# JessicaLeu-code/MotionPlanning_5D_m

Hardware: AMD Instinct MI355X
Metric: CFS iterations/sec, 5-DoF 30-wp 8-obs batch-1024; l_inf wp err vs quadprog (higher is better)
Workload: dtype f64

## Files before the change

### motionplanning_5d_m_amd/csrc/cfs_fused.hip

```cpp
#include "cfs_geom_dev.h"
#include <algorithm>
#include <atomic>
#include <type_traits>

namespace {

#define STAMP_IF(k) if (P.stamps) { const unsigned long long t_ = clock64(); if (tid == 0) s_acc[k] += t_ - t0_; t0_ = t_; }
#define STAMP(k) do { STAMP_IF(k) } while (0)

constexpr int CERT_AT = 6;
#ifndef CFS_WG_PER_CU
#define CFS_WG_PER_CU 1
#endif
constexpr double REF_A = 1e-4;
constexpr double REF_B = 1e-9;
constexpr int MV_BATCH = 16;
#ifndef CFS_TU
#define CFS_TU 8
#endif
#ifndef CFS_PR
#define CFS_PR 64
#endif
static_assert(CFS_PR % 8 == 0 && CFS_PR >= 8, "register-resident P columns come in chunks of 8");
constexpr int FT = 256;
// ... 209 lines not shown
}

template <int PR, int QB>
struct PRow {
    static constexpr int TU = CFS_TU;
    double v[PR];
    __device__ __forceinline__ void zero(double *ptail, int a, int q)
    {
#pragma unroll
        for (int b = 0; b < PR; ++b) v[b] = 0.0;
        for (int b = PR; b < q; ++b) ptail[(b - PR) * QB + a] = 0.0;
    }
    __device__ __forceinline__ double dot(const double *vec, const double *ptail, int a, int q) const
    {
        double s = 0.0;
#pragma unroll
        for (int b0 = 0; b0 < PR; b0 += 8)
            if (b0 < q) {
#pragma unroll
                for (int jj = 0; jj < 8; ++jj) s += v[b0 + jj] * vec[b0 + jj];
                __builtin_amdgcn_sched_barrier(0);
            }
        int b = PR;
        for (; b + TU <= q; b += TU) {
            double t[TU];
#pragma unroll
            for (int jj = 0; jj < TU; ++jj) t[jj] = ptail[(b + jj - PR) * QB + a];
#pragma unroll
            for (int jj = 0; jj < TU; ++jj) s += t[jj] * vec[b + jj];
        }
        for (; b < q; ++b) s += ptail[(b - PR) * QB + a] * vec[b];
        return s;
    }
    __device__ __forceinline__ void axpy(double alpha, const double *vec, double *ptail, int a, int q)
    {
#pragma unroll
        for (int b0 = 0; b0 < PR; b0 += 8)
            if (b0 < q) {
#pragma unroll
                for (int jj = 0; jj < 8; ++jj) v[b0 + jj] += alpha * vec[b0 + jj];
                __builtin_amdgcn_sched_barrier(0);
            }
        int b = PR;
        for (; b + TU <= q; b += TU) {
            double t[TU];
#pragma unroll
            for (int jj = 0; jj < TU; ++jj) t[jj] = ptail[(b + jj - PR) * QB + a];
#pragma unroll
            for (int jj = 0; jj < TU; ++jj) ptail[(b + jj - PR) * QB + a] = t[jj] + alpha * vec[b + jj];
        }
        for (; b < q; ++b) ptail[(b - PR) * QB + a] += alpha * vec[b];
    }
    __device__ __forceinline__ void axpy_mask(double alpha, const double *vec, const double *mask, double *ptail, int a, int q)
    {
#pragma unroll
        for (int b0 = 0; b0 < PR; b0 += 8)
            if (b0 < q) {
#pragma unroll
                for (int jj = 0; jj < 8; ++jj) v[b0 + jj] = (v[b0 + jj] + alpha * vec[b0 + jj]) * mask[b0 + jj];
                __builtin_amdgcn_sched_barrier(0);
            }
        int b = PR;
        for (; b + TU <= q; b += TU) {
            double t[TU];
#pragma unroll
            for (int jj = 0; jj < TU; ++jj) t[jj] = ptail[(b + jj - PR) * QB + a];
#pragma unroll
            for (int jj = 0; jj < TU; ++jj) ptail[(b + jj - PR) * QB + a] = (t[jj] + alpha * vec[b + jj]) * mask[b + jj];
        }
        for (; b < q; ++b) ptail[(b - PR) * QB + a] = (ptail[(b - PR) * QB + a] + alpha * vec[b]) * mask[b];
    }
    __device__ __forceinline__ void set_scaled(double alpha, const double *vec, double *ptail, int a, int q)
    {
#pragma unroll
        for (int b0 = 0; b0 < PR; b0 += 8)
            if (b0 < q) {
#pragma unroll
                for (int jj = 0; jj < 8; ++jj) v[b0 + jj] = alpha * vec[b0 + jj];
                __builtin_amdgcn_sched_barrier(0);
            }
        for (int b = PR; b < q; ++b) ptail[(b - PR) * QB + a] = alpha * vec[b];
    }
    __device__ __forceinline__ void store(double *dst, const double *ptail, int a, int q) const
    {
#pragma unroll
        for (int b0 = 0; b0 < PR; b0 += 8)
            if (b0 < q) {
#pragma unroll
                for (int jj = 0; jj < 8; ++jj) dst[b0 + jj] = v[b0 + jj];
                __builtin_amdgcn_sched_barrier(0);
            }
        int b = PR;
        for (; b + TU <= q; b += TU) {
            double t[TU];
#pragma unroll
            for (int jj = 0; jj < TU; ++jj) t[jj] = ptail[(b + jj - PR) * QB + a];
#pragma unroll
            for (int jj = 0; jj < TU; ++jj) dst[b + jj] = t[jj];
        }
        for (; b < q; ++b) dst[b] = ptail[(b - PR) * QB + a];
    }
};

struct FusedLayout {
    int rb, ob, x, u, qu, g, rhs, xs, up, wb, zb, d, r, rho, lam, prow, act, fre, prev, flag, slot, code, red, small, mx, racc, cost, ptail, lin, y, total_fixed;
};
__host__ __device__ inline FusedLayout fused_layout(int NJ, int H, int nobs, int QB, int PR)
{
    FusedLayout L;
    const int HN = H * NJ, NS = 2 * NJ;
    int o = 0;
    L.rb = o; o += (int)(sizeof(DevRobot) / 8);
    L.ob = o; o += nobs * 6;
    L.x = o; o += H * NS;
    L.u = o; o += HN;
    L.qu = o; o += HN;
    L.g = o; o += nobs * HN;
    L.rhs = o; o += nobs * H;
    L.xs = o; o += 3 * HN;
    L.up = o; o += HN;
    L.act = o; o += (QB + 1) / 2;
    L.fre = o; o += (QB + 1) / 2;
    L.prev = o; o += (QB + 1) / 2;
    L.flag = o; o += (nobs * H + 4 * HN + 7) / 8;
    L.code = o; o += (nobs * H + 4 * HN + 1) / 2;
    L.red = o; o += 64;
    L.small = o; o += 4 * NJ + nobs;
    L.mx = o; o += HN;
    L.racc = o; o += HN;
    L.cost = o; o += (int)(sizeof(DevCost) / 8);
    o = (o + 1) & ~1;
    L.lin = o;
    L.wb = o; o += 3 * HN;
    L.zb = o; o += 3 * HN;
    L.d = o; o += QB;
    L.r = o; o += QB;
    L.rho = o; o += QB;
    L.lam = o; o += QB;
    L.prow = o; o += QB;
    L.slot = o; o += (nobs * H + 4 * HN + 3) / 4;
    L.ptail = o;
    o = (o + 1) & ~1;
    L.y = o;
    L.total_fixed = o;
    return L;
}

template <int NJ, int QB, bool IDENT, bool JAC, class... Soft>
__global__ __launch_bounds__(FT, CFS_WG_PER_CU) void cfs_solve_fused_kernel(FusedParams P, Soft... soft_params)
{
    constexpr bool SOFT = sizeof...(Soft) > 0;
    static_assert(!SOFT || (sizeof...(Soft) == 1 && (std::is_same_v<Soft, SoftParams> && ...)), "Soft is empty or SoftParams");
    const SoftParams S{soft_params...};
    constexpr int NS = 2 * NJ, NVT = nvt(NJ), NE = 2 * NJ + 1;
    extern __shared__ __attribute__((aligned(16))) double lds[];
    const int b = P.order ? P.order[blockIdx.x] : (int)blockIdx.x, tid = threadIdx.x;
    const int H = P.H, nobs = P.nobs, HN = H * NJ, nn = HN, NX = H * NS;
    const double dt = P.dt;
    constexpr int PR = QB < CFS_PR ? QB : CFS_PR;
    const FusedLayout L = fused_layout(NJ, H, nobs, QB, PR);
    DevRobot *rb = reinterpret_cast<DevRobot *>(lds + L.rb);
    double *s_ob = lds + L.ob, *s_x = lds + L.x, *s_u = lds + L.u, *s_qu = lds + L.qu, *s_g = lds + L.g;
    double *s_rhs = lds + L.rhs, *xs = lds + L.xs, *s_up = lds + L.up, *wb = lds + L.wb, *zb = lds + L.zb;
    double *s_d = lds + L.d, *s_r = lds + L.r, *s_rho = lds + L.rho, *s_lam = lds + L.lam, *s_prow = lds + L.prow;
    int *s_act = reinterpret_cast<int *>(lds + L.act);
    int *s_free = reinterpret_cast<int *>(lds + L.fre);
    int *s_prev = reinterpret_cast<int *>(lds + L.prev);
    unsigned char *s_flag = reinterpret_cast<unsigned char *>(lds + L.flag);
    unsigned short *s_slot = reinterpret_cast<unsigned short *>(lds + L.slot);
    int *s_code = reinterpret_cast<int *>(lds + L.code);
    double *red_base = lds + L.red;
    int red_sel = 0;
#define red (red_base + 24 * (red_sel ^= 1))
    double *s_lim = lds + L.small, *s_v0 = s_lim + NJ, *s_th0 = s_v0 + NJ, *s_margin = s_th0 + 2 * NJ;
    double *s_mx = lds + L.mx;
    double *s_racc = lds + L.racc;
    int pool_slot;
    {
        int *pubp = reinterpret_cast<int *>(red_base + 63);
        if (tid == 0) {
            int sidx = (int)(((blockIdx.x * 0x9E3779B1u) >> 8) % (unsigned)P.pool_n);
            int probes = 0;
            while (atomicCAS(&P.pool_flag[sidx * 16], 0, 1) != 0) {
                sidx = sidx + 1 == P.pool_n ? 0 : sidx + 1;
                __builtin_amdgcn_s_sleep(2);
                if (++probes > (1 << 22)) { sidx = -1; break; }
            }
            pubp[0] = sidx;
        }
        __syncthreads();
        pool_slot = pubp[0];
        if (pool_slot < 0) {
            if (tid == 0 && P.piece == 0) { P.status[b] = CFS_NUMERIC; P.iter_O[b] = 1; P.total_iter[b] = 0; }
            return;
        }
    }
    double *const s_pt = P.Pt + (size_t)pool_slot * P.pt_stride;
    double *s_Y = lds + L.y;
    const int QY = P.qy;
    double *const Yg = P.Yg + (size_t)pool_slot * nn * nn;
    auto drop_pool = [&]() {
        __syncthreads();
        if (tid == 0) { __threadfence(); atomicExch(&P.pool_flag[pool_slot * 16], 0); }
    };
    const int ncon = nobs * H + (P.has_bounds ? 4 : 2) * HN;
    const int maxit = 8 * nn + 200;
    for (int e = tid; e < ncon; e += FT) {
        int code;
        if (e < nobs * H) { const int j = e / H; code = mk_code(CT_COL, e - j * H, j); }
        else {
            const int f2 = e - nobs * H, ty = f2 / HN, k = f2 - ty * HN, i = k / NJ;
            code = mk_code(1 + ty, i, k - i * NJ);
        }
        s_code[e] = code;
    }

    {
        const double *src = reinterpret_cast<const double *>(P.rb);
        for (int e = tid; e < (int)(sizeof(DevRobot) / 8); e += FT) lds[L.rb + e] = src[e];
        for (int e = tid; e < nobs * 6; e += FT) s_ob[e] = P.obs[(size_t)b * nobs * 6 + e];
        for (int e = tid; e < NX; e += FT) s_x[e] = P.x_init[(size_t)b * NX + e];
        for (int e = tid; e < HN; e += FT) { s_u[e] = 0.0; s_qu[e] = 0.0; s_mx[e] = P.has_bounds ? P.maxin[e] : 0.0; }
        if (tid < NJ) {
            s_lim[tid] = P.lim[tid];
            s_v0[tid] = P.xR1[(size_t)b * NS + NJ + tid];
            s_th0[tid] = P.xR1[(size_t)b * NS + tid];
        }
        if (tid < nobs) s_margin[tid] = P.margin[tid];
        if (P.cost) {
            const double *csrc = reinterpret_cast<const double *>(P.cost);
            for (int e = tid; e < (int)(sizeof(DevCost) / 8); e += FT) lds[L.cost + e] = csrc[e];
        }
    }
    __syncthreads();
    if (P.has_bounds)
        for (int e = tid; e < HN; e += FT) {
            const int i = e / NJ, c = e - i * NJ;
            double acc = 0.0;
            for (int k = 0; k <= i; ++k) acc += ((double)(i - k) + 0.5) * s_mx[k * NJ + c];
            s_racc[e] = (dt * dt) * acc;
        }
    unsigned long long *s_acc = reinterpret_cast<unsigned long long *>(red_base + 48);
    if (tid < 12) s_acc[tid] = 0ull;
    unsigned long long t0_ = P.stamps ? clock64() : 0ull;
    double cost_new = P.caug[b], cost_old = 100000.0;
    int iter_O = 1, total_iter = 0, noise_row = 0, status = CFS_OK_MAXITER;
    bool done = false;
    const double iw = S.inv_weight;
    int n_soft = 0;
    bool last_soft = false;
    const int nseg = nobs - P.nmesh;
    int launched = 0;
    if (P.resume) {
        for (int e = tid; e < NX; e += FT) s_x[e] = P.x_[(size_t)b * NX + e];
        for (int e = tid; e < HN; e += FT) { s_u[e] = P.u[(size_t)b * nn + e]; s_qu[e] = P.st_qu[(size_t)b * nn + e]; }
        cost_new = P.st_cost[2 * b]; cost_old = P.st_cost[2 * b + 1];
        iter_O = P.iter_O[b]; total_iter = P.total_iter[b]; status = P.status[b];
        noise_row = P.st_noise[b]; done = P.st_done[b] != 0;
        __syncthreads();
    } else if (P.piece == 0) {
        double d2 = 0.0;
        for (int e = tid; e < NX; e += FT) { const double v = s_x[e] - 1.0; d2 += v * v; }
        d2 = block_sum(d2, red, tid);
        if (sqrt(d2) < P.epsilon_O) { done = true; status = CFS_OK_CONVERGED; }
        else if (iter_O > P.max_o_iter) { done = true; status = CFS_OK_MAXITER; }
    } else if (P.piece == 2) {
        for (int e = tid; e < HN; e += FT) s_u[e] = P.u[(size_t)b * nn + e];
        __syncthreads();
    }

    PRow<PR, QB> Pr;
    int prev_q = 0;

    while (!done) {
        bool skip = false;
        if (P.piece == 0 && P.mode == CFS_MODE_PSGCFS) {
            skip = fabs(cost_new - cost_old) < 1e-4;
            if (!skip) cost_old = cost_new;
        } else if (P.piece == 0) cost_old = cost_new;
        const int noise_row_now = noise_row;
        if (P.piece == 0 && P.mode == CFS_MODE_PSGCFS && !skip) ++noise_row;
        auto prep = [&](int ph) {
            if (P.piece == 1) return;
            if (ph == 0) { for (int k = tid; k < HN; k += FT) xs[k] = s_u[k]; }
            else if (ph == 1) roll_lds<NJ>(xs, H, dt, tid);
            else if (ph == 2) {
                const bool psg = P.piece == 0 && P.mode == CFS_MODE_PSGCFS;
                const double sc = (double)iter_O * (double)iter_O + 1.0;
                const bool have = P.noise != nullptr && noise_row_now < P.noise_rows;
                for (int k = tid; k < HN; k += FT) {
                    s_up[k] = xs[2 * HN + k];
                    double v;
                    if (psg && skip) v = s_u[k];
                    else if (psg) {
                        const double nz = have ? P.noise[((size_t)b * P.noise_rows + noise_row_now) * nn + k] : 0.0;
                        v = s_u[k] - P.alpha * ((s_qu[k] + P.ff[(size_t)b * nn + k]) + 10.0 * nz / sc);
                    } else v = P.x0[(size_t)b * nn + k];
                    xs[k] = v;
                }
            } else roll_lds<NJ>(xs, H, dt, tid);
        };
        bool prepped = false;
        if constexpr (JAC) {
            if (nseg > 0) {
                const int W = P.lin_w;
                double *s_sc = lds + L.lin;
                double *s_en = s_sc + W * NJ * 6;
                double *s_tw = s_en + W * NJ * 6;
                double *s_bd = s_en + W * NVT * 6;
                for (int w0 = 0; w0 < H; w0 += W) {
                    const int Wc = min(W, H - w0);
                    if (w0 == 0) prep(0);
                    for (int e = tid; e < Wc * NJ; e += FT) {
                        const int m = e % NJ, wi = e / NJ;
                        double x = s_x[(w0 + wi) * NS + m];
                        x = x - rb->th_off[m];
                        double sn, cs;
                        sincos(x, &sn, &cs);
                        s_sc[e * 2] = sn;
                        s_sc[e * 2 + 1] = cs;
                    }
                    __syncthreads();
                    for (int wi = tid; wi < Wc; wi += FT) arm_chain(rb, NJ, s_sc + wi * NJ * 2, s_en + wi * NJ * 6, s_tw + wi * NJ * 6);
                    if (w0 == 0) prep(1);
                    __syncthreads();
                    STAMP(10);
                    for (int e = tid; e < NJ * Wc * nseg; e += FT) {
                        const int j = e % nseg, wi = (e / nseg) % Wc, k0 = e / (nseg * Wc);
                        s_bd[(wi * NJ + k0) * nseg + j] = seg_seg_dist(s_en + (wi * NJ + k0) * 6, s_ob + j * 6);
                    }
                    if (w0 == 0) prep(2);
                    __syncthreads();
                    STAMP(0);
                    for (int e = tid; e < Wc * nseg; e += FT) {
                        const int j = e % nseg, wi = e / nseg;
                        double m0 = INFINITY;
                        int lk = 0;
#pragma unroll
                        for (int k1 = 1; k1 <= NJ; ++k1) { const double bk = s_bd[(wi * NJ + k1 - 1) * nseg + j]; if (bk < m0) { m0 = bk; lk = k1; } }
                        if (P.dump_linkid && launched == 0) P.dump_linkid[((size_t)b * nobs + j) * H + w0 + wi] = lk;
                        s_rhs[j * H + w0 + wi] = m0;
                        double *g = s_g + (j * H + w0 + wi) * NJ;
                        if (lk > 0) winner_grad(s_en + (wi * NJ + lk - 1) * 6, s_tw + wi * NJ * 6, lk - 1, NJ, s_ob + j * 6, g);
                        else for (int m = 0; m < NJ; ++m) g[m] = 0.0;
                    }
                    if (w0 == 0) { prep(3); prepped = true; }
                    if (w0 + W >= H) __syncthreads();
                    STAMP(11);
                }
            }
        } else {
            if (nseg > 0) {
                const int W = P.lin_w;
                double *s_sc = lds + L.lin;
                double *s_en = s_sc + W * NJ * 6;
                double *s_bd = s_en + W * NVT * 6;
                double *s_dv = s_bd + W * NJ * nseg;
                unsigned short *s_list = reinterpret_cast<unsigned short *>(s_dv + W * nseg * NE);
                int *s_cnt = s_free;
                for (int w0 = 0; w0 < H; w0 += W) {
                    const int Wc = min(W, H - w0);
                    if (w0 == 0) prep(0);
                    for (int e = tid; e < Wc * NJ * 3; e += FT) {
                        const int var = e % 3, m = (e / 3) % NJ, wi = e / (3 * NJ);
                        double x = s_x[(w0 + wi) * NS + m];
                        if (var == 1) x = x + FD_EPS / 2;
                        else if (var == 2) x = x - FD_EPS / 2;
                        x = x - rb->th_off[m];
                        double sn, cs;
                        sincos(x, &sn, &cs);
                        s_sc[((wi * NJ + m) * 3 + var) * 2] = sn;
                        s_sc[((wi * NJ + m) * 3 + var) * 2 + 1] = cs;
                    }
                    __syncthreads();
                    for (int e = tid; e < Wc * NE; e += FT) {
                        const int ev = e % NE, wi = e / NE;
                        double M[12], Mn[12], e6[6];
#pragma unroll
                        for (int k1 = 1; k1 <= NJ; ++k1) {
                            const int avar = (ev == 2 * k1 - 1) ? 1 : (ev >= 2 * k1 ? 2 : 0);
                            const double sn = s_sc[((wi * NJ + k1 - 1) * 3 + avar) * 2], cs = s_sc[((wi * NJ + k1 - 1) * 3 + avar) * 2 + 1];
                            fk_step(rb, k1 - 1, sn, cs, k1 == 1 ? nullptr : M, Mn);
#pragma unroll
                            for (int qq = 0; qq < 12; ++qq) M[qq] = Mn[qq];
                            if (ev <= 2 * k1) {
                                link_ends(rb, k1 - 1, M, e6);
                                double *dstE = s_en + (wi * NVT + kvoff(k1) + ev) * 6;
#pragma unroll
                                for (int qq = 0; qq < 6; ++qq) dstE[qq] = e6[qq];
                            }
                        }
                    }
                    if (w0 == 0) prep(1);
                    __syncthreads();
                    STAMP(10);
                    for (int e = tid; e < NJ * Wc * nseg; e += FT) {
                        const int j = e % nseg, wi = (e / nseg) % Wc, k0 = e / (nseg * Wc);
                        s_bd[(wi * NJ + k0) * nseg + j] = seg_seg_dist(s_en + (wi * NVT + kvoff(k0 + 1)) * 6, s_ob + j * 6);
                    }
                    if (tid < NJ) s_cnt[tid] = 0;
                    if (w0 == 0) prep(2);
                    __syncthreads();
                    for (int e = tid; e < Wc * nseg; e += FT) {
                        const int j = e % nseg, wi = e / nseg;
                        double bk[NJ], m0 = INFINITY;
                        int lk = 0;
#pragma unroll
                        for (int k1 = 1; k1 <= NJ; ++k1) { bk[k1 - 1] = s_bd[(wi * NJ + k1 - 1) * nseg + j]; if (bk[k1 - 1] < m0) { m0 = bk[k1 - 1]; lk = k1; } }
                        if (P.dump_linkid && launched == 0) P.dump_linkid[((size_t)b * nobs + j) * H + w0 + wi] = lk;
                        const double thr = P.no_prune ? INFINITY : fmax(m0, 0.0001) + rb->prune_tol;
#pragma unroll
                        for (int k1 = 1; k1 <= NJ; ++k1)
                            if (bk[k1 - 1] < thr) s_list[(k1 - 1) * W * nseg + atomicAdd(&s_cnt[k1 - 1], 1)] = (unsigned short)((wi << 8) | j);
                        s_dv[e * NE] = m0;
#pragma unroll
                        for (int ev = 1; ev < NE; ++ev) s_dv[e * NE + ev] = INFINITY;
                    }
                    if (w0 == 0) { prep(3); prepped = true; }
                    __syncthreads();
                    STAMP(0);
                    {
                        int offs[NJ + 1];
                        offs[0] = 0;
#pragma unroll
                        for (int k1 = 1; k1 <= NJ; ++k1) offs[k1] = offs[k1 - 1] + s_cnt[k1 - 1] * 2 * k1;
                        for (int e = tid; e < offs[NJ]; e += FT) {
                            int k1 = 1, ent = 0, v = 1;
#pragma unroll
                            for (int kk = 1; kk <= NJ; ++kk)
                                if (e >= offs[kk - 1] && e < offs[kk]) {
                                    const int r_ = e - offs[kk - 1];
                                    k1 = kk; ent = r_ / (2 * kk); v = r_ - ent * (2 * kk) + 1;
                                }
                            const int item = s_list[(k1 - 1) * W * nseg + ent], wi = item >> 8, j = item & 255;
                            const double dis = seg_seg_dist(s_en + (wi * NVT + kvoff(k1) + v) * 6, s_ob + j * 6);
                            double *dv = s_dv + (wi * nseg + j) * NE;
                            const int evhi = (v == 2 * k1) ? NE - 1 : v;
                            for (int ev = v; ev <= evhi; ++ev)
                                __hip_atomic_fetch_min(dv + ev, dis, __ATOMIC_RELAXED, __HIP_MEMORY_SCOPE_WORKGROUP);
                        }
                    }
                    __syncthreads();
                    STAMP(11);
                    for (int e = tid; e < Wc * nseg; e += FT) {
                        const int j = e % nseg, wi = e / nseg;
                        double dev[NE];
#pragma unroll
                        for (int ev = 0; ev < NE; ++ev) dev[ev] = s_dv[e * NE + ev];
                        s_rhs[j * H + w0 + wi] = dev[0];
#pragma unroll
                        for (int m = 0; m < NJ; ++m) s_g[(j * H + w0 + wi) * NJ + m] = (dev[2 * m + 1] - dev[2 * m + 2]) / FD_EPS;
                    }
                    if (w0 + W >= H) __syncthreads();
                }
            }
        }
        if (!prepped && P.piece != 1) {
            prep(0); __syncthreads(); prep(1); __syncthreads(); prep(2); __syncthreads(); prep(3); __syncthreads();
        }

        if (P.nmesh > 0) {
            for (int e = tid; e < P.nmesh * H; e += FT) s_rhs[nseg * H + e] = P.ext_dist[(size_t)b * P.nmesh * H + e];
            for (int e = tid; e < P.nmesh * HN; e += FT) s_g[nseg * HN + e] = P.ext_grad[(size_t)b * P.nmesh * HN + e];
            __syncthreads();
        }

        if (P.dump_dist && launched == 0) {
            for (int e = tid; e < nobs * H; e += FT) P.dump_dist[(size_t)b * nobs * H + e] = s_rhs[e];
            for (int e = tid; e < nobs * HN; e += FT) P.dump_grad[(size_t)b * nobs * HN + e] = s_g[e];
        }
        if (P.piece == 1) { drop_pool(); return; }

        STAMP(0);
        int qp_status = QP_OK, iters = 0;
        int qhi = 0, nfree = 0;
        int npolish = 0;
        auto n_combine = [&](const double *coef, const double *base, int pc_) {
            const int ptype_ = pc_ >> 16, pi_ = (pc_ >> 8) & 0xff, pj_ = pc_ & 0xff;
            const bool two = H <= 32;
            const int lane = two ? (tid & 31) : (tid & 63);
            const int iR = H - 1 - lane;
            const int cstep = two ? 2 * (FT / 64) : FT / 64;
            for (int c = two ? (tid >> 5) : (tid >> 6); c < NJ; c += cstep) {
                double Rp = 0.0, Rv = 0.0;
                if (lane < H) {
                    const int sp_ = s_slot[nobs * H + iR * NJ + c], sm_ = s_slot[nobs * H + HN + iR * NJ + c];
                    for (int j0 = 0; j0 < nobs; j0 += 8) {
                        int sl[8];
#pragma unroll
                        for (int jj = 0; jj < 8; ++jj) sl[jj] = j0 + jj < nobs ? s_slot[(j0 + jj) * H + iR] : 0;
#pragma unroll
                        for (int jj = 0; jj < 8; ++jj)
                            if (sl[jj]) Rp += coef[sl[jj] - 1] * s_g[((j0 + jj) * H + iR) * NJ + c];
                    }
                    if (sp_) Rv -= dt * coef[sp_ - 1];
                    if (sm_) Rv += dt * coef[sm_ - 1];
                }
                const double S1 = two ? half_scan_incl(Rp) : wave_scan_incl(Rp);
                const double cmb = (dt * dt) * S1 + Rv;
                const double S2V = two ? half_scan_incl(cmb) : wave_scan_incl(cmb);
                const double nr_rev = S2V - (0.5 * dt * dt) * S1;
                const int src = (lane < H ? H - 1 - lane : lane) + (two ? (tid & 32) : 0);
                const double nr = __shfl(nr_rev, src, 64);
                double z0 = 0.0;
                if (lane < H) {
                    if (base) z0 = base[lane * NJ + c];
                    else if (ptype_ == CT_COL) z0 = lane <= pi_ ? s_g[(pj_ * H + pi_) * NJ + c] * ((dt * dt) * ((double)(pi_ - lane) + 0.5)) : 0.0;
                    else z0 = (c == pj_ && lane <= pi_) ? (ptype_ == CT_VELP ? -dt : dt) : 0.0;
                    z0 -= nr;
                }
                const double sv = dt * (two ? half_scan_incl(z0) : wave_scan_incl(z0));
                const double spo = dt * (two ? half_scan_incl(sv) : wave_scan_incl(sv)) - (0.5 * dt) * sv;
                if (lane < H) { zb[lane * NJ + c] = z0; zb[HN + lane * NJ + c] = sv; zb[2 * HN + lane * NJ + c] = spo; }
            }
        };
        auto y_combine = [&](const double *coef, const double *base) {
            const int qa = min(qhi, QY);
            for (int k = tid; k < HN; k += FT) {
                double z0 = base ? base[k] : 0.0, z1 = 0.0, z2 = 0.0, z3 = 0.0;
                int a = 0;
                for (; a + 4 <= qa; a += 4) {
                    z0 -= coef[a] * s_Y[a * HN + k];
                    z1 -= coef[a + 1] * s_Y[(a + 1) * HN + k];
                    z2 -= coef[a + 2] * s_Y[(a + 2) * HN + k];
                    z3 -= coef[a + 3] * s_Y[(a + 3) * HN + k];
                }
                for (; a < qa; ++a) z0 -= coef[a] * s_Y[a * HN + k];
                for (a = qa; a + CFS_TU <= qhi; a += CFS_TU) {
                    double t[CFS_TU];
#pragma unroll
                    for (int jj = 0; jj < CFS_TU; ++jj) t[jj] = Yg[(size_t)(a + jj) * nn + k];
#pragma unroll
                    for (int jj = 0; jj < CFS_TU; jj += 4) {
                        z0 -= coef[a + jj] * t[jj]; z1 -= coef[a + jj + 1] * t[jj + 1]; z2 -= coef[a + jj + 2] * t[jj + 2]; z3 -= coef[a + jj + 3] * t[jj + 3];
                    }
                }
                for (; a < qhi; ++a) z0 -= coef[a] * Yg[(size_t)a * nn + k];
                zb[k] = (z0 + z1) + (z2 + z3);
            }
        };
        auto y_combine_roll = [&](const double *coef, const double *base) {
            const int lane = tid & 31;
            for (int c = tid >> 5; c < NJ; c += 2 * (FT / 64)) {
                const int k = lane * NJ + c;
                double z0 = 0.0, z1 = 0.0, z2 = 0.0, z3 = 0.0;
                if (lane < H) {
                    z0 = base ? base[k] : 0.0;
                    int a = 0;
                    for (; a + 4 <= qhi; a += 4) {
                        z0 -= coef[a] * s_Y[a * HN + k];
                        z1 -= coef[a + 1] * s_Y[(a + 1) * HN + k];
                        z2 -= coef[a + 2] * s_Y[(a + 2) * HN + k];
                        z3 -= coef[a + 3] * s_Y[(a + 3) * HN + k];
                    }
                    for (; a < qhi; ++a) z0 -= coef[a] * s_Y[a * HN + k];
                }
                const double z = (z0 + z1) + (z2 + z3);
                const double sv = dt * half_scan_incl(z);
                const double spo = dt * half_scan_incl(sv) - (0.5 * dt) * sv;
                if (lane < H) { zb[k] = z; zb[HN + k] = sv; zb[2 * HN + k] = spo; }
            }
        };
        auto gather_w = [&](int code) {
            const int ptype_ = code >> 16, pi_ = (code >> 8) & 0xff, pj_ = code & 0xff;
            for (int k = tid; k < HN; k += FT) {
                double w0;
                if (ptype_ == CT_COL) {
                    w0 = 0.0;
#pragma unroll
                    for (int cs = 0; cs < NJ; ++cs) {
                        const double gc = s_g[(pj_ * H + pi_) * NJ + cs];
                        w0 += gc * P.M1[(size_t)(pi_ * NJ + cs) * nn + k];
                    }
                } else {
                    const bool vel = ptype_ == CT_VELP || ptype_ == CT_VELM;
                    const double sg = (ptype_ == CT_VELP || ptype_ == CT_BNDP) ? -1.0 : 1.0;
                    w0 = sg * (vel ? P.M2 : P.M3)[(size_t)(pi_ * NJ + pj_) * nn + k];
                }
                wb[k] = w0;
            }
        };
        bool soft = false;
        double viol = 0.0;
        if (!skip) {
            for (int e = tid; e < ncon; e += FT) { s_flag[e] = 0; s_slot[e] = 0; }
            Pr.zero(s_pt, tid, 0);
            if (tid < QB) { s_prev[tid] = s_act[tid]; s_d[tid] = 0.0; s_r[tid] = 0.0; s_rho[tid] = 0.0; s_prow[tid] = 0.0; s_lam[tid] = 0.0; s_act[tid] = -1; }
            for (int e = tid; e < nobs * H; e += FT) {
// ... 482 lines not shown
        for (int k = tid; k < HN; k += FT) {
            const int i = k / NJ, c = k - i * NJ;
            const double un = xs[k], e = s_u[k] - un;
            du2 += e * e;
            const double th = (s_th0[c] + ((double)(i + 1) * dt) * s_v0[c]) + xs[2 * HN + k];
            const double om = s_v0[c] + xs[HN + k];
            const double oth = P.mode == CFS_MODE_PSGCFS ? 1.0 : s_x[i * NS + c];
            const double oom = P.mode == CFS_MODE_PSGCFS ? 1.0 : s_x[i * NS + NJ + c];
            dx2 += (th - oth) * (th - oth) + (om - oom) * (om - oom);
            s_x[i * NS + c] = th;
            s_x[i * NS + NJ + c] = om;
            s_u[k] = un;
            if (P.u_log) P.u_log[((size_t)b * P.max_o_iter + (iter_O - 1)) * nn + k] = un;
            if (P.u_hist) P.u_hist[((size_t)b * P.max_o_iter + (iter_O - 1)) * nn + k] = un;
        }
        double cost = cost_new;
        if (!P.u_hist) {
            if (P.cost) {
                const DevCost *ck = reinterpret_cast<const DevCost *>(lds + L.cost);
                const bool two = H <= 32;
                const int lane = two ? (tid & 31) : (tid & 63), iR = H - 1 - lane;
                const int cstep = two ? 2 * (FT / 64) : FT / 64;
                for (int c = two ? (tid >> 5) : (tid >> 6); c < NJ; c += cstep) {
                    double Rp = 0.0, Rv = 0.0;
                    if (lane < H) {
                        const double wi = iR == H - 1 ? ck->wt : ck->ws;
                        double ap = 0.0, av = 0.0;
#pragma unroll
                        for (int c2 = 0; c2 < NJ; ++c2) {
                            ap += ck->Qp[c + c2 * NJ] * xs[2 * HN + iR * NJ + c2];
                            av += ck->Qv[c + c2 * NJ] * xs[HN + iR * NJ + c2];
                        }
                        Rp = wi * (ap + ck->qc * xs[HN + iR * NJ + c]);
                        Rv = dt * (wi * (ck->qc * xs[2 * HN + iR * NJ + c] + av));
                    }
                    const double S1 = two ? half_scan_incl(Rp) : wave_scan_incl(Rp);
                    const double cmb = (dt * dt) * S1 + Rv;
                    const double S2V = two ? half_scan_incl(cmb) : wave_scan_incl(cmb);
                    const double y_rev = S2V - (0.5 * dt * dt) * S1;
                    const int src = (lane < H ? H - 1 - lane : lane) + (two ? (tid & 32) : 0);
                    const double y = __shfl(y_rev, src, 64);
                    if (lane < H) {
                        const int k = lane * NJ + c;
                        double ru = 0.0;
#pragma unroll
                        for (int c2 = 0; c2 < NJ; ++c2) ru += ck->Rs[c + c2 * NJ] * xs[lane * NJ + c2];
                        const double sq = y + ru;
                        s_qu[k] = sq;
                        cpart += xs[k] * (0.5 * sq + P.ff[(size_t)b * nn + k]);
                    }
                }
            } else
            for (int k = tid; k < HN; k += FT) {
                double sa[8] = {0.0, 0.0, 0.0, 0.0, 0.0, 0.0, 0.0, 0.0};
                int c = 0;
                for (; c + MV_BATCH <= HN; c += MV_BATCH) {
                    double ld[MV_BATCH];
#pragma unroll
                    for (int j = 0; j < MV_BATCH; ++j) ld[j] = P.QQ[k + (size_t)(c + j) * nn];
#pragma unroll
                    for (int j = 0; j < MV_BATCH; ++j) sa[j & 7] += ld[j] * xs[c + j];
                }
                for (; c < HN; ++c) sa[0] += P.QQ[k + (size_t)c * nn] * xs[c];
                const double s = ((sa[0] + sa[1]) + (sa[2] + sa[3])) + ((sa[4] + sa[5]) + (sa[6] + sa[7]));
                s_qu[k] = s;
                cpart += xs[k] * (0.5 * s + P.ff[(size_t)b * nn + k]);
            }
        }
        block_sum3(du2, dx2, cpart, red, tid);
        if (P.u_hist) {
            if (tid == 0) P.e_u_all[(size_t)b * P.max_o_iter + (iter_O - 1)] = sqrt(du2);
        } else {
            cost = cpart + P.caug[b];
            if (tid == 0) {
                const size_t o = (size_t)b * P.max_o_iter + (iter_O - 1);
                P.cost_all[o] = cost;
                P.e_cost_all[o] = fabs(cost_old - cost);
                P.e_u_all[o] = sqrt(du2);
            }
        }
        STAMP(9);
        cost_new = cost;
        ++iter_O;
        if (sqrt(dx2) < P.epsilon_O) { done = true; status = CFS_OK_CONVERGED; }
        else if (iter_O > P.max_o_iter) { done = true; status = CFS_OK_MAXITER; }
        if (P.max_launch_iters > 0 && ++launched >= P.max_launch_iters) break;
    }

    drop_pool();
    __syncthreads();
    for (int e = tid; e < HN; e += FT) P.u[(size_t)b * nn + e] = s_u[e];
    for (int e = tid; e < NX; e += FT) P.x_[(size_t)b * NX + e] = s_x[e];
    if constexpr (SOFT) {
        if (last_soft && (status == CFS_OK_CONVERGED || status == CFS_OK_MAXITER)) status = CFS_SOFT_ENDED;
        if (tid == 0 && S.n_soft) S.n_soft[b] = n_soft;
    }
    if (tid == 0) { P.iter_O[b] = iter_O; P.total_iter[b] = total_iter; P.status[b] = status; }
    if (P.st_qu) {
        for (int e = tid; e < HN; e += FT) P.st_qu[(size_t)b * nn + e] = s_qu[e];
        if (tid == 0) { P.st_cost[2 * b] = cost_new; P.st_cost[2 * b + 1] = cost_old; P.st_noise[b] = noise_row; P.st_done[b] = done ? 1 : 0; }
    }
    if (P.stamps && tid == 0) for (int k = 0; k < 12; ++k) P.stamps[(size_t)b * 12 + k] = s_acc[k];
}

#undef red

template <int NJ, int QB, bool IDENT, bool JAC, bool SOFT>
hipError_t launch_fused_inst2(const FusedParams &p, size_t lds, hipStream_t s, const SoftParams *sp)
{
    static std::atomic<unsigned long long> attr_set{0ull};
    using Kernel = std::conditional_t<SOFT, void (*)(FusedParams, SoftParams), void (*)(FusedParams)>;
    const Kernel kern = cfs_solve_fused_kernel<NJ, QB, IDENT, JAC>;
    int dev = 0;
    hipError_t e = hipGetDevice(&dev);
    if (e != hipSuccess) return e;
    if (dev >= 64 || !((attr_set.load(std::memory_order_acquire) >> dev) & 1ull)) {
        e = hipFuncSetAttribute(reinterpret_cast<const void *>(kern), hipFuncAttributeMaxDynamicSharedMemorySize, 160 * 1024);
        if (e != hipSuccess) return e;
        if (dev < 64) attr_set.fetch_or(1ull << dev, std::memory_order_release);
    }
    if constexpr (SOFT) hipLaunchKernelGGL(kern, dim3(p.B), dim3(FT), lds, s, p, *sp);
    else hipLaunchKernelGGL(kern, dim3(p.B), dim3(FT), lds, s, p);
    return hipGetLastError();
}

#ifndef CFS_IDENT_SET
#define CFS_IDENT_SET 2
#endif
template <int NJ, int QB, bool JAC, bool SOFT>
hipError_t launch_fused_inst(const FusedParams &p, size_t lds, hipStream_t s, const SoftParams *sp)
{
    const bool ident = p.mode == CFS_MODE_PSGCFS;
#if CFS_IDENT_SET != 0
    if (ident) return launch_fused_inst2<NJ, QB, true, JAC, SOFT>(p, lds, s, sp);
#endif
#if CFS_IDENT_SET != 1
    if (!ident) return launch_fused_inst2<NJ, QB, false, JAC, SOFT>(p, lds, s, sp);
#endif
    return hipErrorInvalidValue;
}

struct FusedPlan {
    int nn, QB;
    FusedLayout L;
    size_t avail, per_wp;
};
FusedPlan fused_plan(int nj, int H, int nobs)
{
    FusedPlan q;
    q.nn = H * nj;
    q.QB = q.nn <= 96 ? 96 : (q.nn <= 160 ? 160 : 256);
    q.L = fused_layout(nj, H, nobs, q.QB, q.QB < CFS_PR ? q.QB : CFS_PR);
    q.avail = (160 * 1024 / CFS_WG_PER_CU) / 8 - 64;
    q.per_wp = (size_t)nj * 6 + (size_t)nvt(nj) * 6 + (size_t)nj * nobs + (size_t)nobs * (2 * nj + 1) + ((size_t)nj * nobs + 3) / 4;
    return q;
}

}

template <FusedTier T>
bool fused_fits_tier(int nj, int H, int nobs)
{
    const FusedPlan q = fused_plan(nj, H, nobs);
    return (size_t)q.L.total_fixed + (size_t)4 * q.nn <= q.avail && (size_t)q.L.lin + q.per_wp <= q.avail;
}

template <FusedTier T, bool JAC, bool SOFT>
hipError_t launch_fused_tier(int nj, FusedParams p, hipStream_t s, const SoftParams *sp)
{
    const FusedPlan q = fused_plan(nj, p.H, p.nobs);
    const int nn = q.nn;
    const FusedLayout &L = q.L;
    const bool ident = p.mode == CFS_MODE_PSGCFS;
    if ((size_t)L.total_fixed + (ident ? 0 : 4 * nn) > q.avail) return hipErrorInvalidValue;
    const size_t region = q.avail - L.total_fixed;
    int qy = ident ? 0 : (int)(region / nn);
    if (qy > nn) qy = nn;
    int w = (int)((q.avail - L.lin) / q.per_wp);
    if (w < 1) return hipErrorInvalidValue;
    w = (p.H + (p.H + w - 1) / w - 1) / ((p.H + w - 1) / w);
    p.qy = qy;
    p.lin_w = w;
    const size_t need = std::max((size_t)L.total_fixed + (size_t)qy * nn, (size_t)L.lin + (size_t)w * q.per_wp);
    const size_t lds = need * 8;
    switch (nj * 1000 + q.QB) {
    case 2096: return launch_fused_inst<2, 96, JAC, SOFT>(p, lds, s, sp);
    case 3096: return launch_fused_inst<3, 96, JAC, SOFT>(p, lds, s, sp);
    case 4096: return launch_fused_inst<4, 96, JAC, SOFT>(p, lds, s, sp);
    case 5096: return launch_fused_inst<5, 96, JAC, SOFT>(p, lds, s, sp);
    case 6096: return launch_fused_inst<6, 96, JAC, SOFT>(p, lds, s, sp);
    case 2160: return launch_fused_inst<2, 160, JAC, SOFT>(p, lds, s, sp);
    case 4160: return launch_fused_inst<4, 160, JAC, SOFT>(p, lds, s, sp);
    case 5160: return launch_fused_inst<5, 160, JAC, SOFT>(p, lds, s, sp);
    case 6160: return launch_fused_inst<6, 160, JAC, SOFT>(p, lds, s, sp);
    case 3160: return launch_fused_inst<3, 160, JAC, SOFT>(p, lds, s, sp);
    case 3256: return launch_fused_inst<3, 256, JAC, SOFT>(p, lds, s, sp);
    case 4256: return launch_fused_inst<4, 256, JAC, SOFT>(p, lds, s, sp);
    case 5256: return launch_fused_inst<5, 256, JAC, SOFT>(p, lds, s, sp);
    case 6256: return launch_fused_inst<6, 256, JAC, SOFT>(p, lds, s, sp);
    default: return hipErrorInvalidValue;
    }
}

template hipError_t launch_fused_tier<CFS_TIER, CFS_JAC, CFS_SOFT>(int, FusedParams, hipStream_t, const SoftParams *);
#if !CFS_JAC && !CFS_SOFT
template bool fused_fits_tier<CFS_TIER>(int, int, int);
#endif
```

Before: 10.69 million.

## Recompute perturbed forward kinematics on demand instead of storing all variant link endpoints

The finite-difference Jacobian path used to precompute and store link endpoints for every perturbation variant (NVT entries per waypoint) in LDS. Now only the nominal endpoints are stored, and the narrow-phase loop recomputes the perturbed forward-kinematics chain for each surviving (link, variant, obstacle) candidate. The per-waypoint LDS footprint shrinks, which could allow larger windows or better occupancy. The cost is redundant FK work per candidate pair. The analytic-Jacobian path's LDS offsets are also tightened.

```diff
diff --git a/motionplanning_5d_m_amd/csrc/cfs_fused.hip b/motionplanning_5d_m_amd/csrc/cfs_fused.hip
--- a/motionplanning_5d_m_amd/csrc/cfs_fused.hip
+++ b/motionplanning_5d_m_amd/csrc/cfs_fused.hip
@@ -385,7 +385,7 @@
     constexpr bool SOFT = sizeof...(Soft) > 0;
     static_assert(!SOFT || (sizeof...(Soft) == 1 && (std::is_same_v<Soft, SoftParams> && ...)), "Soft is empty or SoftParams");
     const SoftParams S{soft_params...};
-    constexpr int NS = 2 * NJ, NVT = nvt(NJ), NE = 2 * NJ + 1;
+    constexpr int NS = 2 * NJ, NE = 2 * NJ + 1;
     extern __shared__ __attribute__((aligned(16))) double lds[];
     const int b = P.order ? P.order[blockIdx.x] : (int)blockIdx.x, tid = threadIdx.x;
     const int H = P.H, nobs = P.nobs, HN = H * NJ, nn = HN, NX = H * NS;
@@ -538,9 +538,9 @@
             if (nseg > 0) {
                 const int W = P.lin_w;
                 double *s_sc = lds + L.lin;
-                double *s_en = s_sc + W * NJ * 6;
+                double *s_en = s_sc + W * NJ * 2;
                 double *s_tw = s_en + W * NJ * 6;
-                double *s_bd = s_en + W * NVT * 6;
+                double *s_bd = s_tw + W * NJ * 6;
                 for (int w0 = 0; w0 < H; w0 += W) {
                     const int Wc = min(W, H - w0);
                     if (w0 == 0) prep(0);
@@ -587,7 +587,7 @@
                 const int W = P.lin_w;
                 double *s_sc = lds + L.lin;
                 double *s_en = s_sc + W * NJ * 6;
-                double *s_bd = s_en + W * NVT * 6;
+                double *s_bd = s_en + W * NJ * 6;
                 double *s_dv = s_bd + W * NJ * nseg;
                 unsigned short *s_list = reinterpret_cast<unsigned short *>(s_dv + W * nseg * NE);
                 int *s_cnt = s_free;
@@ -606,22 +606,15 @@
                         s_sc[((wi * NJ + m) * 3 + var) * 2 + 1] = cs;
                     }
                     __syncthreads();
-                    for (int e = tid; e < Wc * NE; e += FT) {
-                        const int ev = e % NE, wi = e / NE;
-                        double M[12], Mn[12], e6[6];
+                    for (int wi = tid; wi < Wc; wi += FT) {
+                        double M[12], Mn[12];
 #pragma unroll
                         for (int k1 = 1; k1 <= NJ; ++k1) {
-                            const int avar = (ev == 2 * k1 - 1) ? 1 : (ev >= 2 * k1 ? 2 : 0);
-                            const double sn = s_sc[((wi * NJ + k1 - 1) * 3 + avar) * 2], cs = s_sc[((wi * NJ + k1 - 1) * 3 + avar) * 2 + 1];
+                            const double sn = s_sc[(wi * NJ + k1 - 1) * 6], cs = s_sc[(wi * NJ + k1 - 1) * 6 + 1];
                             fk_step(rb, k1 - 1, sn, cs, k1 == 1 ? nullptr : M, Mn);
 #pragma unroll
                             for (int qq = 0; qq < 12; ++qq) M[qq] = Mn[qq];
-                            if (ev <= 2 * k1) {
-                                link_ends(rb, k1 - 1, M, e6);
-                                double *dstE = s_en + (wi * NVT + kvoff(k1) + ev) * 6;
-#pragma unroll
-                                for (int qq = 0; qq < 6; ++qq) dstE[qq] = e6[qq];
-                            }
+                            link_ends(rb, k1 - 1, M, s_en + (wi * NJ + k1 - 1) * 6);
                         }
                     }
                     if (w0 == 0) prep(1);
@@ -629,7 +622,7 @@
                     STAMP(10);
                     for (int e = tid; e < NJ * Wc * nseg; e += FT) {
                         const int j = e % nseg, wi = (e / nseg) % Wc, k0 = e / (nseg * Wc);
-                        s_bd[(wi * NJ + k0) * nseg + j] = seg_seg_dist(s_en + (wi * NVT + kvoff(k0 + 1)) * 6, s_ob + j * 6);
+                        s_bd[(wi * NJ + k0) * nseg + j] = seg_seg_dist(s_en + (wi * NJ + k0) * 6, s_ob + j * 6);
                     }
                     if (tid < NJ) s_cnt[tid] = 0;
                     if (w0 == 0) prep(2);
@@ -666,7 +659,22 @@
                                     k1 = kk; ent = r_ / (2 * kk); v = r_ - ent * (2 * kk) + 1;
                                 }
                             const int item = s_list[(k1 - 1) * W * nseg + ent], wi = item >> 8, j = item & 255;
-                            const double dis = seg_seg_dist(s_en + (wi * NVT + kvoff(k1) + v) * 6, s_ob + j * 6);
+                            double M[12], e6[6];
+                            {
+                                const int avar = v == 1 ? 1 : (v >= 2 ? 2 : 0);
+                                fk_step(rb, 0, s_sc[(wi * NJ * 3 + avar) * 2], s_sc[(wi * NJ * 3 + avar) * 2 + 1], nullptr, M);
+                            }
+#pragma unroll 1
+                            for (int kk = 2; kk <= k1; ++kk) {
+                                const int avar = (v == 2 * kk - 1) ? 1 : (v >= 2 * kk ? 2 : 0);
+                                const double sn = s_sc[((wi * NJ + kk - 1) * 3 + avar) * 2], cs = s_sc[((wi * NJ + kk - 1) * 3 + avar) * 2 + 1];
+                                double Mn[12];
+                                fk_step(rb, kk - 1, sn, cs, M, Mn);
+#pragma unroll
+                                for (int qq = 0; qq < 12; ++qq) M[qq] = Mn[qq];
+                            }
+                            link_ends(rb, k1 - 1, M, e6);
+                            const double dis = seg_seg_dist(e6, s_ob + j * 6);
                             double *dv = s_dv + (wi * nseg + j) * NE;
                             const int evhi = (v == 2 * k1) ? NE - 1 : v;
                             for (int ev = v; ev <= evhi; ++ev)
@@ -1455,7 +1463,7 @@
     q.QB = q.nn <= 96 ? 96 : (q.nn <= 160 ? 160 : 256);
     q.L = fused_layout(nj, H, nobs, q.QB, q.QB < CFS_PR ? q.QB : CFS_PR);
     q.avail = (160 * 1024 / CFS_WG_PER_CU) / 8 - 64;
-    q.per_wp = (size_t)nj * 6 + (size_t)nvt(nj) * 6 + (size_t)nj * nobs + (size_t)nobs * (2 * nj + 1) + ((size_t)nj * nobs + 3) / 4;
+    q.per_wp = (size_t)nj * 6 + (size_t)nj * 6 + (size_t)nj * nobs + (size_t)nobs * (2 * nj + 1) + ((size_t)nj * nobs + 3) / 4;
     return q;
 }
 
```

Result: slower. 10.49 million (median of 2 runs) (-1.9%).
